# VideoVerses/VideoTuna-dev

Hardware: AMD Instinct MI355X
Metric: finetune samples/sec, CogVideoX-2B T2V LoRA 49x480x720 bf16 (higher is better)
Workload: dtype bf16; 1 GPU; CogVideoX-2B T2V LoRA finetune 49x480x720 (configs[1]): latents [4,13,16,60,90], text [4,226,4096], r=4 LoRA on to_q/k/v/out, 4 samples per optimizer step as in the YAML (batch_size 2 x accumulate_grad_batches 2), run as 1 micro-batch(es) of 4; mode=lora, model=CogVideoX-2B, micro_batch=4, accumulate_grad_batches=1, global_batch=4, seq_len=17776, layers=30, parallelism=dp1, recompute=none (107 GB of block activations kept in HBM), weights=seeded random init (no checkpoints offline), text=pre-encoded prompt embeddings (synthetic), latents=pre-encoded latents (synthetic)

## Files before the change

### include/vt355.h

```cpp
#ifndef VT355_H
#define VT355_H
#ifdef __cplusplus
extern "C" {
#endif

#define VT_OK 0
#define VT_ERR_BAD_SHAPE (-1)
#define VT_ERR_BAD_ALIGN (-2)
#define VT_ERR_LAUNCH (-3)
#define VT_ERR_UNSUPPORTED (-4)

int vt_version(void);
const char* vt_arch(void);
const char* vt_error_string(int code);

#define VT_EPI_BIAS 0
#define VT_EPI_BIAS_GELU 1
#define VT_EPI_GATED_RES 2
#define VT_EPI_DGELU 3

int vt_gemm_bf16(const void* A, int lda, const void* W, int ldw, void* C, int ldc,
                 int M, int N, int K, const void* bias, int epilogue, int out_fp32,
                 const void* R, int ldr, int r_mod,
                 const float* gate_txt, const float* gate_vid, int gate_bstride, int S, int St,
                 void* C2, int ldc2, const void* U, int ldu, void* stream);
int vt_gemm_set_tile(int mode);
int vt_gemm_bf16_kernel(int M, int N, int K);
int vt_conv_set_tile(int mode);

int vt_gemm_nt_bf16(const void* A, int lda, const void* B, int ldb, float* C, int ldc, int M, int P, int Q,
                    float alpha, int accumulate, void* stream);
int vt_gemm_nt_bf16_unpad(const void* A, int lda, const void* B, int ldb, float* C, int ldc, int M, int P, int Q,
                          float alpha, int accumulate, int row_group, int row_keep, int col_group, int col_keep, void* stream);

int vt_group_colsum(const void* X, int ldx, const void* Y, int ldy, const float* mean, const float* rstd,
                    float* out1, float* out2, long long M, int D, int S, int St, int grouped,
                    long long o_bstride, long long o_segstride, void* stream);

int vt_qk_ln_param_grads(const float* dq_hat, int lddq, const void* dk_hat, int lddk, const void* qkv, int ld,
                         const float* mean, const float* rstd, float* out_2x2x64, long long M, int H,
                         const float* rope_cos, const float* rope_sin, int S, int St, void* stream);
int vt_ln_param_combine(const float* G1, const float* G2, int G, int D, const void* gamma, const void* beta,
                        const float* scale_txt, const float* scale_vid, int bstride, float* dgamma, float* dbeta,
                        float* dshift_txt, float* dshift_vid, float* dscale_txt, float* dscale_vid, int dbstride,
                        int grouped, void* stream);
int vt_small_linear_bwd(const float* dy, int ldy, const void* x, int ldx, const void* W, float* dW, float* db,
                        float* dx, int lddx, int Bn, int N, int K, void* stream);
int vt_silu_bwd(const float* dy, const void* x, float* dx, long long n, void* stream);

int vt_attn_fwd_hd64(const void* q, const void* k, const void* v, void* o, float* lse2,
                     int B, int H, int S,
                     long long q_rs, long long k_rs, long long v_rs, long long o_rs,
                     long long q_bs, long long k_bs, long long v_bs, long long o_bs,
                     float softmax_scale, int q_prescaled, void* stream);

int vt_attn_fwd_bias_hd64(const void* q, const void* k, const void* v, const float* bias_t, void* o, float* lse2,
                          int B, int H, int S,
                          long long q_rs, long long k_rs, long long v_rs, long long o_rs,
                          long long q_bs, long long k_bs, long long v_bs, long long o_bs,
                          float softmax_scale, void* stream);
int vt_gemm_splitk_f32(const void* A, int lda, const void* W, int ldw, float* C, int ldc, int M, int N, int K, int splits, void* stream);
int vt_residual_cast_bf16(const float* acc, long long lda, const void* R, long long ldr, void* out, long long ldo, long long M, int N,
                          void* stream);
long long vt_groupnorm_ws_bytes(int N, int C);
int vt_groupnorm_silu_cl(const void* x, long long ldx, const void* gamma, const void* beta, void* y, long long ldy,
                         int N, long long P, int C, int G, float eps, int silu, float* ws, long long ws_bytes, void* stream);
int vt_causal_conv3d_cl(const void* x, long long ldx, const void* wk, const void* bias, const void* res, long long ldr,
                        void* y, long long ldy, int N, int T, int H, int W, int Cin, int Cout, void* stream);
int vt_downsample_conv2d_cl(const void* x, long long ldx, const void* wk, const void* bias, void* y, long long ldy,
                            int N, int T, int H, int W, int Cin, int Cout, void* stream);
int vt_causal_conv3d_in8_cl(const void* x, const void* wk, const void* bias, void* y, long long ldy,
                            int N, int T, int H, int W, int Cout, void* stream);
int vt_temporal_pool_cl(const void* x, long long ldx, void* y, long long ldy, int N, int T, long long HW, int C, int keep_first,
                        void* stream);
int vt_rmsnorm_bf16(const void* x, long long ldx, const void* w, void* y, long long ldy, long long M, int D, float eps,
                    void* stream);
int vt_gated_gelu_bf16(const void* u, long long ldu, void* y, long long ldy, long long M, int F, void* stream);

int vt_attn_bwd_hd64(const void* q, const void* k, const void* v, const void* o, const void* dout,
                     const float* lse2, float* delta_ws, float* dq_f32, void* dk, void* dv,
                     int B, int H, int S,
                     long long q_rs, long long k_rs, long long v_rs, long long o_rs, long long do_rs,
                     long long dq_rs, long long dk_rs, long long dv_rs,
                     long long q_bs, long long k_bs, long long v_bs, long long o_bs, long long do_bs,
                     long long dq_bs, long long dk_bs, long long dv_bs,
                     float softmax_scale, int q_prescaled, void* chain_ws, long long chain_ws_bytes, void* stream);
long long vt_attn_bwd_chain_ws_bytes(int B, int H, int S);
int vt_attn_bwd_set_chain(int chain_len, int slots);

int vt_ln_modulate_fwd(const void* x, int ldx, void* y, int ldy, const void* gamma, const void* beta,
                       const float* shift_txt, const float* scale_txt, const float* shift_vid,
                       const float* scale_vid, int mod_bstride, float* mean, float* rstd,
                       int M, int D, int S, int St, float eps, void* stream);
int vt_ln_modulate_bwd(const void* dy, int lddy, const void* x, int ldx, const float* mean, const float* rstd,
                       const void* gamma, const float* scale_txt, const float* scale_vid, int mod_bstride,
                       const void* dres, int lddres, void* dx, int lddx,
                       int M, int D, int S, int St, void* stream);

int vt_qk_layernorm_fwd(const void* qkv, int ld, void* out, int ldo, const void* gq, const void* bq,
                        const void* gk, const void* bk, float* mean, float* rstd,
                        long long M, int H, float eps, float q_scale,
                        const float* rope_cos, const float* rope_sin, int S, int St, void* stream);
int vt_qk_layernorm_bwd(const float* dq_hat, int lddq, const void* dk_hat, int lddk, const void* qkv, int ld,
                        const float* mean, const float* rstd, const void* gq, const void* gk,
                        void* dqkv, int ldd, long long M, int H,
                        const float* rope_cos, const float* rope_sin, int S, int St, void* stream);

int vt_gate_mul(const void* x, int ldx, void* y, int ldy, const float* g_txt, const float* g_vid, int bstride,
                long long M, int D, int S, int St, void* stream);
int vt_silu_bf16(const void* x, void* y, long long n, void* stream);
// ... 212 lines not shown
```

### videotuna-dev_amd/_lib.py

```python
import ctypes as C
import os

_HERE = os.path.dirname(os.path.abspath(__file__))
_LIB = None


class VtError(RuntimeError):
    pass


def lib_path() -> str:
    return os.environ.get("VT355_LIB") or os.path.join(_HERE, "libvt355.so")


_vp, _i, _ll, _f, _fp = C.c_void_p, C.c_int, C.c_longlong, C.c_float, C.c_void_p
PROTOTYPES = {
    "vt_version": [],
    "vt_arch": [],
    "vt_error_string": [_i],
    "vt_gemm_bf16": [_vp, _i, _vp, _i, _vp, _i, _i, _i, _i, _vp, _i, _i, _vp, _i, _i, _fp, _fp, _i, _i, _i,
                     _vp, _i, _vp, _i, _vp],
    "vt_gemm_set_tile": [_i],
    "vt_gemm_bf16_kernel": [_i, _i, _i],
    "vt_conv_set_tile": [_i],
    "vt_transpose_bf16": [_vp, _ll, _ll, _vp, _ll, _ll, _i, _i, _i, _vp],
    "vt_transpose_multi_bf16": [_vp, _i, _ll, _vp],
    "vt_gemm_nt_bf16": [_vp, _i, _vp, _i, _fp, _i, _i, _i, _i, _f, _i, _vp],
    "vt_gemm_nt_bf16_unpad": [_vp, _i, _vp, _i, _fp, _i, _i, _i, _i, _f, _i, _i, _i, _i, _i, _vp],
    "vt_group_colsum": [_vp, _i, _vp, _i, _fp, _fp, _fp, _fp, _ll, _i, _i, _i, _i, _ll, _ll, _vp],
    "vt_qk_ln_param_grads": [_fp, _i, _vp, _i, _vp, _i, _fp, _fp, _fp, _ll, _i, _fp, _fp, _i, _i, _vp],
    "vt_ln_param_combine": [_fp, _fp, _i, _i, _vp, _vp, _fp, _fp, _i, _fp, _fp, _fp, _fp, _fp, _fp, _i, _i, _vp],
    "vt_small_linear_bwd": [_fp, _i, _vp, _i, _vp, _fp, _fp, _fp, _i, _i, _i, _i, _vp],
    "vt_silu_bwd": [_fp, _vp, _fp, _ll, _vp],
    "vt_attn_fwd_hd64": [_vp, _vp, _vp, _vp, _fp, _i, _i, _i, _ll, _ll, _ll, _ll, _ll, _ll, _ll, _ll, _f, _i, _vp],
    "vt_attn_fwd_bias_hd64": [_vp, _vp, _vp, _fp, _vp, _fp, _i, _i, _i, _ll, _ll, _ll, _ll, _ll, _ll, _ll, _ll, _f, _vp],
    "vt_gemm_splitk_f32": [_vp, _i, _vp, _i, _fp, _i, _i, _i, _i, _i, _vp],
    "vt_residual_cast_bf16": [_fp, _ll, _vp, _ll, _vp, _ll, _ll, _i, _vp],
    "vt_groupnorm_ws_bytes": [_i, _i],
    "vt_groupnorm_silu_cl": [_vp, _ll, _vp, _vp, _vp, _ll, _i, _ll, _i, _i, _f, _i, _fp, _ll, _vp],
    "vt_causal_conv3d_cl": [_vp, _ll, _vp, _vp, _vp, _ll, _vp, _ll, _i, _i, _i, _i, _i, _i, _vp],
    "vt_causal_conv3d_in8_cl": [_vp, _vp, _vp, _vp, _ll, _i, _i, _i, _i, _i, _vp],
    "vt_downsample_conv2d_cl": [_vp, _ll, _vp, _vp, _vp, _ll, _i, _i, _i, _i, _i, _i, _vp],
    "vt_temporal_pool_cl": [_vp, _ll, _vp, _ll, _i, _i, _ll, _i, _i, _vp],
    "vt_rmsnorm_bf16": [_vp, _ll, _vp, _vp, _ll, _ll, _i, _f, _vp],
    "vt_gated_gelu_bf16": [_vp, _ll, _vp, _ll, _ll, _i, _vp],
    "vt_attn_bwd_hd64": [_vp, _vp, _vp, _vp, _vp, _fp, _fp, _fp, _vp, _vp, _i, _i, _i,
                         _ll, _ll, _ll, _ll, _ll, _ll, _ll, _ll, _ll, _ll, _ll, _ll, _ll, _ll, _ll, _ll, _f, _i, _vp, _ll, _vp],
    "vt_attn_bwd_chain_ws_bytes": [_i, _i, _i],
    "vt_attn_bwd_set_chain": [_i, _i],
    "vt_ln_modulate_fwd": [_vp, _i, _vp, _i, _vp, _vp, _fp, _fp, _fp, _fp, _i, _fp, _fp, _i, _i, _i, _i, _f, _vp],
    "vt_ln_modulate_bwd": [_vp, _i, _vp, _i, _fp, _fp, _vp, _fp, _fp, _i, _vp, _i, _vp, _i, _i, _i, _i, _i, _vp],
    "vt_qk_layernorm_fwd": [_vp, _i, _vp, _i, _vp, _vp, _vp, _vp, _fp, _fp, _ll, _i, _f, _f, _fp, _fp, _i, _i, _vp],
    "vt_qk_layernorm_bwd": [_fp, _i, _vp, _i, _vp, _i, _fp, _fp, _vp, _vp, _vp, _i, _ll, _i, _fp, _fp, _i, _i, _vp],
    "vt_gate_mul": [_vp, _i, _vp, _i, _fp, _fp, _i, _ll, _i, _i, _i, _vp],
    "vt_silu_bf16": [_vp, _vp, _ll, _vp],
    "vt_cast_f32_bf16": [_fp, _vp, _ll, _vp],
    "vt_timestep_embedding": [_vp, _vp, _i, _i, _i, _f, _vp],
    "vt_patchify": [_vp, _vp, _i, _i, _i, _i, _i, _i, _i, _vp],
    "vt_unpatchify": [_vp, _vp, _i, _i, _i, _i, _i, _i, _i, _vp],
    "vt_add_noise": [_fp, _fp, _fp, _fp, _vp, _ll, _i, _vp],
    "vt_diffusion_loss": [_vp, _vp, _fp, _fp, _fp, _fp, _fp, _fp, _vp, _ll, _i, _f, _vp],
    "vt_diffusion_loss_bwd": [_vp, _vp, _fp, _fp, _fp, _fp, _fp, _vp, _ll, _i, _vp],
    "vt_adamw": [_fp, _fp, _fp, _fp, _vp, _ll, _f, _f, _f, _f, _f, _i, _f, _vp, _vp],
    "vt_grad_sqnorm_partials": [],
    "vt_grad_sqnorm": [_fp, _ll, _fp, _i, _vp],
    "vt_clip_finalize": [_fp, _i, _f, _f, _fp, _vp],
    "vt_adamw_clip": [_fp, _fp, _fp, _fp, _vp, _ll, _f, _f, _f, _f, _f, _i, _f, _vp, _fp, _f, _vp],
    "vt_lora_down": [_vp, _i, _vp, _i, _i, _vp, _i, _ll, _i, _i, _vp],
    "vt_skinny_tn": [_vp, _i, _vp, _i, _i, _fp, _ll, _ll, _f, _ll, _i, _fp, _vp],
    "vt_skinny_tn_workspace_bytes": [_i],
    "vt_lora_up_add": [_vp, _i, _vp, _i, _vp, _i, _i, _ll, _i, _vp],
    "vt_lora_pack_b": [_fp, _vp, _i, _i, _i, _i, _f, _vp],
    "vt_lora_pack_bt": [_fp, _vp, _i, _i, _i, _i, _f, _vp],
    "vt_lora_down_wide": [_vp, _i, _vp, _i, _i, _i, _i, _i, _vp, _i, _ll, _i, _vp],
    "vt_lora_tn_wide": [_vp, _i, _vp, _i, _i, _fp, _ll, _ll, _f, _ll, _i, _vp],
    "vt_lora_up_add_wide": [_vp, _i, _vp, _i, _vp, _i, _i, _i, _i, _ll, _i, _vp],
    "vt_lora_pack_b_wide": [_fp, _vp, _i, _i, _i, _i, _i, _i, _f, _vp],
    "vt_lora_pack_bt_wide": [_fp, _vp, _i, _i, _i, _i, _i, _i, _f, _vp],
    "vt_lora_down_drop": [_vp, _i, _vp, _i, _i, _i, _vp, _i, _ll, _i, _i, _f, C.c_ulonglong, _i, _vp],
    "vt_skinny_tn_drop": [_vp, _i, _vp, _i, _i, _i, _fp, _ll, _ll, _f, _ll, _i, _fp, _f, C.c_ulonglong, _i, _vp],
    "vt_lora_up_add_drop": [_vp, _i, _vp, _i, _vp, _i, _i, _i, _ll, _i, _f, C.c_ulonglong, _i, _vp],
    "vt_lora_down_wide_drop_fits": [_i, _i],
    "vt_lora_down_wide_drop": [_vp, _i, _vp, _i, _i, _i, _i, _i, _vp, _i, _ll, _i, _f, C.c_ulonglong, _i, _vp],
    "vt_lora_tn_wide_drop": [_vp, _i, _vp, _i, _i, _fp, _ll, _ll, _f, _ll, _i, _f, C.c_ulonglong, _i, _vp],
    "vt_lora_up_add_wide_drop": [_vp, _i, _vp, _i, _vp, _i, _i, _i, _i, _ll, _i, _f, C.c_ulonglong, _i, _vp],
    "vt_lora_up_add_dgelu_drop": [_vp, _i, _vp, _i, _vp, _i, _i, _i, _vp, _i, _ll, _i, _f, C.c_ulonglong, _i, _vp],
    "vt_lora_up_add_wide_dgelu_drop": [_vp, _i, _vp, _i, _vp, _i, _i, _i, _i, _vp, _i, _ll, _i, _f, C.c_ulonglong, _i, _vp],
    "vt_lora_down_wide_drop_at": [_vp, _i, _vp, _i, _i, _i, _i, _i, _vp, _i, _ll, _i, _f, C.c_ulonglong, _i] + [_ll] * 5 + [_i, _i, _vp],
    "vt_lora_tn_wide_drop_at": [_vp, _i, _vp, _i, _i, _fp, _ll, _ll, _f, _ll, _i, _f, C.c_ulonglong, _i] + [_ll] * 5 + [_i, _i, _vp],
    "vt_lora_up_add_wide_drop_at": [_vp, _i, _vp, _i, _vp, _i, _i, _i, _i, _ll, _i, _f, C.c_ulonglong, _i] + [_ll] * 5 + [_i, _i, _vp],
    "vt_lora_up_add_wide_dgelu_drop_at": [_vp, _i, _vp, _i, _vp, _i, _i, _i, _i, _vp, _i, _ll, _i, _f, C.c_ulonglong, _i] + [_ll] * 5
                                         + [_i, _i, _vp],
    "vt_dora_norm": [_vp, _i, _vp, _i, _vp, _i, _i, _i, _i, _f, _fp, _fp, _vp],
    "vt_dora_scale": [_vp, _ll, _vp, _ll, _fp, _i, _i, _i, _vp],
    "vt_dora_transpose_scale": [_vp, _ll, _vp, _ll, _fp, _i, _i, _vp],
    "vt_dora_db_add": [_fp, _fp, _fp, _i, _i, _vp],
    "vt_dora_dm": [_fp, _fp, _vp, _fp, _fp, _i, _vp],
    "vt_conv_cl": [_vp, _ll, _vp, _vp, _fp, _i, _vp, _ll, _vp, _ll] + [_i] * 13 + [_vp],
    "vt_conv_dw_cl": [_vp, _ll, _vp, _ll, _fp] + [_i] * 13 + [_i, _vp],
    "vt_conv_dw_bias_cl": [_vp, _ll, _vp, _ll, _fp, _fp] + [_i] * 13 + [_i, _vp],
    "vt_conv_desc_extents": [_ll, _ll] + [_i] * 11 + [C.POINTER(C.c_longlong)] * 3,
    "vt_groupnorm_silu_bwd_cl": [_vp, _ll, _vp, _ll, _vp, _fp, _fp, _ll, _vp, _ll, _fp, _fp, _i, _ll, _i, _i, _i, _i, _vp],
    "vt_geglu_fwd": [_vp, _ll, _vp, _ll, _ll, _i, _vp],
    "vt_geglu_bwd": [_vp, _ll, _vp, _ll, _vp, _ll, _ll, _i, _vp],
    "vt_add_rows_bf16": [_vp, _ll, _vp, _ll, _vp, _ll, _ll, _i, _vp],
# ... 60 lines not shown
```

### videotuna-dev_amd/csrc/gemm_bf16.hip

```cpp
#include "gemm_epilogue.h"

#define BM 128
#define BN 128
#define BK 64
#define CS_LD 132

template <int EPI, bool OUT_F32>
__global__ __launch_bounds__(256, 2) void gemm_tn_kernel(GemmParams p) {
    __shared__ __attribute__((aligned(16))) char smem[65536];
    const int tid = threadIdx.x, lane = tid & 63, wave = tid >> 6;
    const int wm = wave & 1, wn = wave >> 1;
    const int nbm = (p.M + BM - 1) / BM, nbn = (p.N + BN - 1) / BN;
    const int id = xcd_remap(blockIdx.x, nbm * nbn);
    const int GM = 8;
    const int in_group = GM * nbn;
    const int group = id / in_group;
    const int first_m = group * GM;
    const int gsz = min(nbm - first_m, GM);
    const int tile_m = first_m + (id % in_group) % gsz;
    const int tile_n = (id % in_group) / gsz;
    const int row0 = tile_m * BM, col0 = tile_n * BN;

    const long long a_rem = (long long)(p.M - row0) * p.lda * 2;
    const long long w_rem = (long long)(p.N - col0) * p.ldw * 2;
// ... 36 lines not shown
        if (kt + 1 < nk) dma(kt + 1, buf ^ 1);
        const char* As = smem + buf * 32768;
        const char* Ws = As + 16384;
#pragma unroll
        for (int ks = 0; ks < 2; ++ks) {
            const int coff = (((ks * 4 + fq) ^ fx) << 4);
            bf16x8 af[4], wf[4];
#pragma unroll
            for (int t = 0; t < 4; ++t) {
                af[t] = *(const bf16x8*)(As + (wm * 64 + t * 16 + frow) * 128 + coff);
                wf[t] = *(const bf16x8*)(Ws + (wn * 64 + t * 16 + frow) * 128 + coff);
            }
#pragma unroll
            for (int tn = 0; tn < 4; ++tn)
#pragma unroll
                for (int tm = 0; tm < 4; ++tm)
                    acc[tn][tm] = __builtin_amdgcn_mfma_f32_16x16x32_bf16(wf[tn], af[tm], acc[tn][tm], 0, 0, 0);
        }
        __syncthreads();
    }

    float* Cs = (float*)smem;
    const int er = tid >> 5;
    const int ec = (tid & 31) * 4;
    const int n = col0 + ec;
    float bias4[4] = {0.f, 0.f, 0.f, 0.f};
    if (p.bias != nullptr && n < p.N) {
#pragma unroll
        for (int j = 0; j < 4; ++j) bias4[j] = bf2f(p.bias[n + j]);
    }
#pragma unroll
    for (int half = 0; half < 2; ++half) {
        if (wm == half) {
#pragma unroll
            for (int tn = 0; tn < 4; ++tn)
#pragma unroll
                for (int tm = 0; tm < 4; ++tm) {
                    int ml = tm * 16 + frow;
                    int nl = wn * 64 + tn * 16 + fq * 4;
                    *(f32x4*)(Cs + ml * CS_LD + nl) = acc[tn][tm];
                }
        }
        __syncthreads();
#pragma unroll
        for (int pass = 0; pass < 8; ++pass) {
            const int ml = pass * 8 + er;
            const int m = row0 + half * 64 + ml;
            if (m < p.M && n < p.N) {
                f32x4 v = *(const f32x4*)(Cs + ml * CS_LD + ec);
                gemm_epilogue_store<EPI, OUT_F32>(p, m, n, v, bias4);
            }
        }
        __syncthreads();
    }
}

template <int EPI, bool F32>
static int launch(const GemmParams& p, hipStream_t st) {
    const int nbm = (p.M + BM - 1) / BM, nbn = (p.N + BN - 1) / BN;
    hipLaunchKernelGGL((gemm_tn_kernel<EPI, F32>), dim3(nbm * nbn), dim3(256), 0, st, p);
    return hipGetLastError() == hipSuccess ? VT_OK : VT_ERR_LAUNCH;
}

static bool al16(const void* p) { return (((uintptr_t)p) & 15) == 0; }

int vt_gemm_big_dispatch(const GemmParams& p, int epilogue, int out_fp32, hipStream_t st);
int vt_gemm_pc_dispatch(const GemmParams& p, int epilogue, int out_fp32, hipStream_t st);
static int g_gemm_tile = 0;
extern "C" int vt_gemm_set_tile(int mode) {
    if (mode < 0 || mode > 3) return VT_ERR_BAD_SHAPE;
    g_gemm_tile = mode;
    return VT_OK;
}
static int pick_tile(int M, int N, int K) {
    const int mode = g_gemm_tile;
    if (mode) return mode;
    const long long t256 = (long long)((M + 255) / 256) * ((N + 255) / 256);
    const long long tpc = (long long)((M + 255) / 256) * ((N + 127) / 128);
    if (N >= 6144 && t256 >= 512) return 2;
    if (K >= 512 && M >= 1024) {
        const long long passes = (t256 + 255) / 256;
        const bool full = t256 <= 256 ? t256 >= 160 : 10 * t256 >= 9 * passes * 256;
        if (full && (N >= 2560 || ((N % 640) == 0 && N <= 1280) || ((N % 256) >= 192 && K >= 4096))) return 2;
    }
    if (tpc >= 512 && K >= 512) return 3;
    if (M > 64 && M <= 1024 && (long long)N * K >= (1LL << 24)) return 3;
    return 1;
}

int vt_gemm_pc_bm(int M);
extern "C" int vt_gemm_bf16_kernel(int M, int N, int K) {
    if (M <= 0 || N <= 0 || K <= 0) return VT_ERR_BAD_SHAPE;
    const int tile = pick_tile(M, N, K);
    return tile == 3 && vt_gemm_pc_bm(M) == 128 ? 4 : tile;
}

extern "C" int vt_gemm_bf16(const void* A, int lda, const void* W, int ldw, void* C, int ldc,
                            int M, int N, int K, const void* bias, int epilogue, int out_fp32,
                            const void* R, int ldr, int r_mod,
                            const float* gate_txt, const float* gate_vid, int gate_bstride, int S, int St,
                            void* C2, int ldc2, const void* U, int ldu, void* stream) {
    if (M <= 0 || N <= 0 || K <= 0 || (K % BK) != 0 || (N % 4) != 0) return VT_ERR_BAD_SHAPE;
    if ((lda % 8) || (ldw % 8) || (ldc % 4) || lda < K || ldw < K || ldc < N) return VT_ERR_BAD_SHAPE;
    if (!al16(A) || !al16(W) || !al16(C)) return VT_ERR_BAD_ALIGN;
    GemmParams p;
    p.A = (const bf16_t*)A; p.W = (const bf16_t*)W; p.C = C; p.bias = (const bf16_t*)bias;
    p.R = (const bf16_t*)R; p.gate_txt = gate_txt; p.gate_vid = gate_vid;
    p.C2 = (bf16_t*)C2; p.U = (const bf16_t*)U;
    p.M = M; p.N = N; p.K = K; p.lda = lda; p.ldw = ldw; p.ldc = ldc; p.ldr = ldr; p.ldc2 = ldc2; p.ldu = ldu;
    p.S = S > 0 ? S : 1; p.St = St; p.gate_bstride = gate_bstride; p.r_mod = r_mod; p.splits = 1;
    hipStream_t st = (hipStream_t)stream;
    const int tile = pick_tile(M, N, K);
    const bool big = tile == 2;
    if (tile == 3) {
        if (epilogue == EPI_BIAS_GELU && (out_fp32 || C2 == nullptr || (ldc2 % 4) || !al16(C2))) return VT_ERR_BAD_SHAPE;
        if (epilogue == EPI_GATED_RES && (out_fp32 || R == nullptr || (ldr % 4) || !al16(R))) return VT_ERR_BAD_SHAPE;
        if (epilogue == EPI_DGELU && (out_fp32 || U == nullptr || (ldu % 4) || !al16(U))) return VT_ERR_BAD_SHAPE;
        return vt_gemm_pc_dispatch(p, epilogue, out_fp32, st);
    }
    switch (epilogue) {
        case EPI_BIAS:
            if (big) return vt_gemm_big_dispatch(p, epilogue, out_fp32, st);
            return out_fp32 ? launch<EPI_BIAS, true>(p, st) : launch<EPI_BIAS, false>(p, st);
        case EPI_BIAS_GELU:
            if (out_fp32 || C2 == nullptr || (ldc2 % 4) || !al16(C2)) return VT_ERR_BAD_SHAPE;
            if (big) return vt_gemm_big_dispatch(p, epilogue, 0, st);
            return launch<EPI_BIAS_GELU, false>(p, st);
        case EPI_GATED_RES:
            if (out_fp32 || R == nullptr || (ldr % 4) || !al16(R)) return VT_ERR_BAD_SHAPE;
            if (C2 != nullptr && ((ldc2 % 4) || !al16(C2))) return VT_ERR_BAD_SHAPE;
            if (gate_vid != nullptr && (gate_txt == nullptr || (gate_bstride % 4) || !al16(gate_vid) || !al16(gate_txt)))
                return VT_ERR_BAD_SHAPE;
            if (big) return vt_gemm_big_dispatch(p, epilogue, 0, st);
            return launch<EPI_GATED_RES, false>(p, st);
        case EPI_DGELU:
            if (out_fp32 || U == nullptr || (ldu % 4) || !al16(U)) return VT_ERR_BAD_SHAPE;
            if (big) return vt_gemm_big_dispatch(p, epilogue, 0, st);
            return launch<EPI_DGELU, false>(p, st);
        default:
            return VT_ERR_UNSUPPORTED;
    }
}
```

### videotuna-dev_amd/csrc/gemm_big_bf16.hip

```cpp
#include "gemm_epilogue.h"

#define GB_BM 256
#define GB_BN 256
#define GB_BK 64
#define GB_STAGE 65536
#define GB_CS_LD 260

typedef int gb_i32x4 __attribute__((ext_vector_type(4)));

__device__ __forceinline__ gb_i32x4 gb_words(const void* base, unsigned bytes) {
    const unsigned long long a = (unsigned long long)base;
    return (gb_i32x4){(int)(unsigned)a, (int)((a >> 32) & 0xffffu), (int)bytes, 0x00020000};
}

template <int EPI, bool OUT_F32>
__global__ __launch_bounds__(512, 1) void gemm_tn_big_kernel(GemmParams p) {
    __shared__ __attribute__((aligned(16))) char smem[2 * GB_STAGE];
    const int tid = threadIdx.x, lane = tid & 63;
    const int wave = __builtin_amdgcn_readfirstlane(tid >> 6);
    const int wm = wave & 1, wn = wave >> 1;
    const int nbm = (p.M + GB_BM - 1) / GB_BM, nbn = (p.N + GB_BN - 1) / GB_BN;
    const int ntiles = nbm * nbn;
    const int spx = gridDim.x >> 3;
    const int slot = (int)(blockIdx.x & 7) * spx + (int)(blockIdx.x >> 3);
    const unsigned smem_lds = (unsigned)(uintptr_t)(__attribute__((address_space(3))) char*)smem;

    const int drl = lane >> 3, dcp = lane & 7;
    const int row0p = 8 * wave + drl;
    const int sw = (row0p >> 1) & 7;
    const int a_voff0 = row0p * p.lda * 2 + ((dcp ^ sw) << 4);
    const int w_voff0 = row0p * p.ldw * 2 + ((dcp ^ sw) << 4);
    const int a_pstep = 64 * p.lda * 2, w_pstep = 64 * p.ldw * 2;
    auto dma = [&](const GemmTile& t, int kt, int buf) {
        const int soff = kt * GB_BK * 2;
        __amdgpu_buffer_rsrc_t ra = make_rsrc(t.a, t.a_bytes), rw = make_rsrc(t.w, t.w_bytes);
#pragma unroll
        for (int j = 0; j < 4; ++j) {
            char* dst = smem + buf * GB_STAGE + (wave + 8 * j) * 1024;
            __builtin_amdgcn_raw_ptr_buffer_load_lds(ra, (__attribute__((address_space(3))) void*)dst, 16, a_voff0, soff + j * a_pstep, 0, 0);
            __builtin_amdgcn_raw_ptr_buffer_load_lds(rw, (__attribute__((address_space(3))) void*)(dst + 32768), 16, w_voff0, soff + j * w_pstep, 0, 0);
        }
    };
    auto dma_hidden = [&](const GemmTile& t, int buf) {
        const gb_i32x4 ra = gb_words(t.a, t.a_bytes), rw = gb_words(t.w, t.w_bytes);
#pragma unroll
        for (int j = 0; j < 4; ++j) {
            const unsigned dst = smem_lds + buf * GB_STAGE + (wave + 8 * j) * 1024;
            asm volatile("s_mov_b32 m0, %0\n\ts_nop 0\n\tbuffer_load_dwordx4 %1, %2, %3 offen lds" :: "s"(dst), "v"(a_voff0), "s"(ra), "s"(j * a_pstep) : "memory");
            asm volatile("s_mov_b32 m0, %0\n\ts_nop 0\n\tbuffer_load_dwordx4 %1, %2, %3 offen lds" :: "s"(dst + 32768), "v"(w_voff0), "s"(rw), "s"(j * w_pstep) : "memory");
        }
    };

    const int nk = p.K / GB_BK;
    const int fr16 = lane & 15, fq = lane >> 4, fx16 = (fr16 >> 1) & 7;
    const int er = tid >> 6;
    const int ec = (tid & 63) * 4;

    if (slot >= ntiles) return;
    GemmTile cur = gemm_tile<GB_BM, GB_BN>(p, slot, nbm, nbn);
    int buf = 0;
    dma(cur, 0, 0);
    for (int tile = slot; tile < ntiles; tile += gridDim.x) {
        const bool has_next = tile + (int)gridDim.x < ntiles;
        GemmTile nxt = cur;
        if (has_next) nxt = gemm_tile<GB_BM, GB_BN>(p, tile + gridDim.x, nbm, nbn);

        f32x4 acc16[4][8];
#pragma unroll
        for (int i = 0; i < 4; ++i)
#pragma unroll
            for (int j = 0; j < 8; ++j) acc16[i][j] = (f32x4){0.f, 0.f, 0.f, 0.f};

        __syncthreads();
        for (int kt = 0; kt < nk; ++kt) {
            const bool last = kt + 1 == nk;
            auto issue = [&]() {
                if (!last) dma(cur, kt + 1, buf ^ 1);
                else if (has_next) dma_hidden(nxt, buf ^ 1);
            };
            const bool late = wave >= 4;
            if (!late) issue();
            const char* As = smem + buf * GB_STAGE + (wm * 128 + fr16) * 128;
            const char* Ws = smem + buf * GB_STAGE + 32768 + (wn * 64 + fr16) * 128;
#pragma unroll
            for (int ks = 0; ks < 2; ++ks) {
                if (ks == 1 && late) issue();
                const int coff = (((ks * 4 + fq) ^ fx16) << 4);
                bf16x8 af[8], wf[4];
#pragma unroll
                for (int t = 0; t < 8; ++t) af[t] = *(const bf16x8*)(As + t * 2048 + coff);
#pragma unroll
                for (int t = 0; t < 4; ++t) wf[t] = *(const bf16x8*)(Ws + t * 2048 + coff);
#pragma unroll
                for (int tm = 0; tm < 8; ++tm)
#pragma unroll
                    for (int tn = 0; tn < 4; ++tn)
                        acc16[tn][tm] = __builtin_amdgcn_mfma_f32_16x16x32_bf16(wf[tn], af[tm], acc16[tn][tm], 0, 0, 0);
            }
            if (!last) __syncthreads();
            else gemm_lds_barrier();
            buf ^= 1;
        }

        float* Cs = (float*)(smem + (buf ^ 1) * GB_STAGE);
        const int n = cur.col0 + ec;
        float bias4[4] = {0.f, 0.f, 0.f, 0.f};
        if (p.bias != nullptr && n < p.N) {
#pragma unroll
            for (int j = 0; j < 4; ++j) bias4[j] = bf2f(p.bias[n + j]);
        }
        constexpr bool HAS_AUX = EPI == EPI_GATED_RES || EPI == EPI_DGELU;
        u32x2 aux[4], auxn[4];
        auto aux_fetch = [&](int slab, u32x2* dst) {
#pragma unroll
            for (int pass = 0; pass < 4; ++pass) {
                const int m = cur.row0 + slab * 32 + pass * 8 + er;
                dst[pass] = (u32x2){0u, 0u};
                if (HAS_AUX && wave < 8 && m < p.M && n < p.N) dst[pass] = gemm_epilogue_aux_load<EPI>(p, m, n);
            }
        };
        aux_fetch(0, aux);
        GateCtx gctx;
        if (EPI == EPI_GATED_RES) gctx = gate_ctx_load(p, cur.row0, GB_BM, n);
#pragma unroll
        for (int slab = 0; slab < 8; ++slab) {
            if (wave < 8 && wm == (slab >> 2)) {
#pragma unroll
                for (int t2 = 0; t2 < 2; ++t2)
#pragma unroll
                    for (int tn = 0; tn < 4; ++tn)
                        *(f32x4*)(Cs + (t2 * 16 + fr16) * GB_CS_LD + wn * 64 + tn * 16 + 4 * fq) = acc16[tn][(slab & 3) * 2 + t2];
            }
            gemm_lds_barrier();
            if (slab < 7) aux_fetch(slab + 1, auxn);
#pragma unroll
            for (int pass = 0; pass < 4; ++pass) {
                const int ml = pass * 8 + er;
                const int m = cur.row0 + slab * 32 + ml;
                if (wave < 8 && m < p.M && n < p.N) {
                    const f32x4 v = *(const f32x4*)(Cs + ml * GB_CS_LD + ec);
                    gemm_epilogue_store_aux<EPI, OUT_F32>(p, m, n, v, bias4, aux[pass], EPI == EPI_GATED_RES ? &gctx : nullptr);
                }
            }
            gemm_lds_barrier();
#pragma unroll
            for (int pass = 0; pass < 4; ++pass) aux[pass] = auxn[pass];
        }
        cur = nxt;
    }
}

template <int EPI, bool F32>
static int launch_big(const GemmParams& p, hipStream_t st) {
    const int nbm = (p.M + GB_BM - 1) / GB_BM, nbn = (p.N + GB_BN - 1) / GB_BN;
    static int slots = 0;
    if (slots == 0) {
        int dev = 0, cus = 0;
        if (hipGetDevice(&dev) != hipSuccess || hipDeviceGetAttribute(&cus, hipDeviceAttributeMultiprocessorCount, dev) != hipSuccess) cus = 0;
        slots = cus >= 8 ? cus / 8 * 8 : 8;
    }
    const int ntiles = nbm * nbn;
    const int grid = ntiles < slots ? (ntiles + 7) / 8 * 8 : slots;
    hipLaunchKernelGGL((gemm_tn_big_kernel<EPI, F32>), dim3(grid), dim3(512), 0, st, p);
    return hipGetLastError() == hipSuccess ? VT_OK : VT_ERR_LAUNCH;
}

int vt_gemm_big_dispatch(const GemmParams& p, int epilogue, int out_fp32, hipStream_t st) {
    switch (epilogue) {
        case EPI_BIAS:
            return out_fp32 ? launch_big<EPI_BIAS, true>(p, st) : launch_big<EPI_BIAS, false>(p, st);
        case EPI_BIAS_GELU: return launch_big<EPI_BIAS_GELU, false>(p, st);
        case EPI_GATED_RES: return launch_big<EPI_GATED_RES, false>(p, st);
        case EPI_DGELU: return launch_big<EPI_DGELU, false>(p, st);
        default: return VT_ERR_UNSUPPORTED;
    }
}
```

### videotuna-dev_amd/ops.py

```python
from __future__ import annotations

import math
import os
from typing import Optional

import torch

from ._lib import check, load_library

BF16 = torch.bfloat16
EPI_BIAS, EPI_BIAS_GELU, EPI_GATED_RES, EPI_DGELU = 0, 1, 2, 3


def _stream() -> int:
    return torch.cuda.current_stream().cuda_stream


_PROFILE = {"on": False, "events": {}, "work": {}}
_PROFILED = ("attn_fwd", "attn_bwd", "conv", "conv_dw")


def profile_reset(on: bool):
    _PROFILE["on"] = on
    if on:
# ... 304 lines not shown
    check(load_library().vt_downsample_conv2d_cl(x.data_ptr(), x.stride(3), wk.data_ptr(), _p(bias), y.data_ptr(), y.stride(3),
                                                 N, T, H, W, Cin, Cout, _stream()), "vt_downsample_conv2d_cl")
    return y


def temporal_pool_frames(T: int, keep_first: bool) -> int:
    return 1 + (T - 1) // 2 if keep_first else T // 2


def temporal_pool(x, y, keep_first: bool = True):
    _req(x, BF16, "x", 5); _req(y, BF16, "y", 5)
    N, T, H, W, C = x.shape
    To = temporal_pool_frames(T, keep_first)
    if tuple(y.shape) != (N, To, H, W, C) or To < 1:
        raise ValueError(f"y must be {(N, To, H, W, C)}, got {tuple(y.shape)}")
    _cl_check(x, "x"); _cl_check(y, "y")
    check(load_library().vt_temporal_pool_cl(x.data_ptr(), x.stride(3), y.data_ptr(), y.stride(3), N, T, H * W, C, int(keep_first),
                                             _stream()), "vt_temporal_pool_cl")
    return y


def rmsnorm(x, w, y, eps: float = 1e-6):
    _req(x, BF16, "x", 2); _req(y, BF16, "y", 2); _req(w, BF16, "w", 1)
    check(load_library().vt_rmsnorm_bf16(x.data_ptr(), x.stride(0), w.data_ptr(), y.data_ptr(), y.stride(0), x.shape[0], x.shape[1],
                                         eps, _stream()), "vt_rmsnorm_bf16")


def gated_gelu(u, y):
    _req(u, BF16, "u", 2); _req(y, BF16, "y", 2)
    check(load_library().vt_gated_gelu_bf16(u.data_ptr(), u.stride(0), y.data_ptr(), y.stride(0), u.shape[0], y.shape[1], _stream()),
          "vt_gated_gelu_bf16")


def attn_bwd_chain_workspace(B: int, H: int, S: int, device) -> Optional[torch.Tensor]:
    if _SIDE_STREAMS["n"] > 0 or _CHAIN_STATE["disabled"]:
        return None
    n = int(load_library().vt_attn_bwd_chain_ws_bytes(B, H, S))
    if n <= 0:
        return None
    key = str(device)
    ws = _CHAIN_WS.get(key)
    if ws is None or ws.numel() < n:
        old = ws
        ws = _CHAIN_WS[key] = torch.empty(n, dtype=torch.uint8, device=device)
        ws[:256].zero_()
        if old is not None:
            ws[64:256].copy_(old[64:256])
    return ws


_CHAIN_WS = {}
_SIDE_STREAMS = {"n": 0}
_CHAIN_STATE = {"disabled": False, "redone": 0, "verify": __import__("os").environ.get("VT355_CHAIN_VERIFY", "launch")}


def attn_bwd_chain_redone() -> int:
    return _CHAIN_STATE["redone"]


def declare_side_stream(active: bool):
    _SIDE_STREAMS["n"] = max(0, _SIDE_STREAMS["n"] + (1 if active else -1))


def chain_guard(device) -> Optional[torch.Tensor]:
    ws = _CHAIN_WS.get(str(device))
    return None if ws is None else ws[64:68].view(torch.int32)


def attn_bwd_chain_errors() -> int:
    return sum(int(ws[64:68].view(torch.int32).item()) for ws in _CHAIN_WS.values())


def attn_bwd_chain_errors_clear():
    for ws in _CHAIN_WS.values():
        ws[64:256].zero_()


def conv_set_tile(mode: int = 0):
    check(load_library().vt_conv_set_tile(mode), "vt_conv_set_tile")


def gemm_set_tile(mode: int = 0):
    check(load_library().vt_gemm_set_tile(mode), "vt_gemm_set_tile")


def gemm_kernel(M: int, N: int, K: int) -> int:
    k = load_library().vt_gemm_bf16_kernel(M, N, K)
    if k < 0:
        check(k, "vt_gemm_bf16_kernel")
    return k


def attn_bwd_set_chain(chain_len: int = 0, slots: int = 0):
    check(load_library().vt_attn_bwd_set_chain(chain_len, slots), "vt_attn_bwd_set_chain")


def attn_bwd_chain_error(chain_ws: torch.Tensor) -> int:
    return int(chain_ws[32:36].view(torch.int32).item())


def attn_bwd(q, k, v, o, do, lse2, delta_ws, dq_f32, dk, dv, B: int, H: int, S: int, scale: Optional[float] = None,
             q_prescaled: bool = False, chain_ws: Optional[torch.Tensor] = None, _entry=None):
    scale = 1.0 / math.sqrt(64) if scale is None else scale
    for n, t in (("q", q), ("k", k), ("v", v), ("o", o), ("do", do), ("dk", dk), ("dv", dv)):
        _req(t, BF16, n, 3)
    _req(dq_f32, torch.float32, "dq_f32", 3)
    lib = load_library()

    def launch(ws, fn=None):
        check((fn or lib.vt_attn_bwd_hd64)(q.data_ptr(), k.data_ptr(), v.data_ptr(), o.data_ptr(), do.data_ptr(),
                               lse2.data_ptr(), delta_ws.data_ptr(), dq_f32.data_ptr(), dk.data_ptr(), dv.data_ptr(),
                               B, H, S,
                               q.stride(1), k.stride(1), v.stride(1), o.stride(1), do.stride(1),
                               dq_f32.stride(1), dk.stride(1), dv.stride(1),
                               q.stride(0), k.stride(0), v.stride(0), o.stride(0), do.stride(0),
                               dq_f32.stride(0), dk.stride(0), dv.stride(0), scale, int(q_prescaled),
                               None if ws is None else ws.data_ptr(), 0 if ws is None else ws.numel(),
                               _stream()),
          "vt_attn_bwd_hd64")
    with _timed("attn_bwd"):
        launch(chain_ws, _entry)
    if chain_ws is not None and _CHAIN_STATE["verify"] == "launch" and attn_bwd_chain_error(chain_ws) != 0:
        import warnings
        _CHAIN_STATE["disabled"] = True
        _CHAIN_STATE["redone"] += 1
        warnings.warn("vt_attn_bwd_hd64: a dQ hand-off wait timed out (the persistent workgroups were not all resident: another stream or a "
                      "profiler shared the CUs); the launch was redone with plain atomics and the hand-off chains are switched off for the rest "
                      "of this process (VT_BWD_CHAIN=1 avoids them from the start; ops.declare_side_stream(True) announces a concurrent stream)")
        dq_f32.zero_()
        launch(None)
        chain_ws[32:36].zero_()
        chain_ws[64:68].zero_()


def ln_modulate_fwd(x, y, gamma, beta, mod, mean, rstd, D: int, S: int, St: int, eps: float):
    _req(x, BF16, "x", 2); _req(y, BF16, "y", 2)
    m = (None, None, None, None, 0) if mod is None else mod
    lib = load_library()
    with _timed_hbm("ln_modulate_fwd", x.shape[0], 4.0 * x.shape[0] * D):
        check(lib.vt_ln_modulate_fwd(x.data_ptr(), x.stride(0), y.data_ptr(), y.stride(0), _p(gamma), _p(beta),
                                     _p(m[0]), _p(m[1]), _p(m[2]), _p(m[3]), m[4], _p(mean), _p(rstd),
                                     x.shape[0], D, S, St, eps, _stream()), "vt_ln_modulate_fwd")


def ln_modulate_bwd(dy, x, mean, rstd, gamma, scales, dres, dx, D: int, S: int, St: int):
    _req(dy, BF16, "dy", 2); _req(x, BF16, "x", 2); _req(dx, BF16, "dx", 2)
    sc = (None, None, 0) if scales is None else scales
    lib = load_library()
    with _timed_hbm("ln_modulate_bwd", x.shape[0], (6.0 if dres is None else 8.0) * x.shape[0] * D):
        check(lib.vt_ln_modulate_bwd(dy.data_ptr(), dy.stride(0), x.data_ptr(), x.stride(0), mean.data_ptr(), rstd.data_ptr(),
                                     _p(gamma), _p(sc[0]), _p(sc[1]), sc[2], _p(dres), 0 if dres is None else dres.stride(0),
                                     dx.data_ptr(), dx.stride(0), x.shape[0], D, S, St, _stream()), "vt_ln_modulate_bwd")


def qk_layernorm_fwd(qkv, out, gq, bq, gk, bk, mean, rstd, H: int, eps: float, q_scale: float = 1.0, rope=None):
    _req(qkv, BF16, "qkv", 2); _req(out, BF16, "out", 2)
    lib = load_library()
    rc, rsn, S, St = _rope_args(rope, qkv.shape[0])
    with _timed_hbm("qk_layernorm_fwd", qkv.shape[0], 8.0 * qkv.shape[0] * H * 64):
        check(lib.vt_qk_layernorm_fwd(qkv.data_ptr(), qkv.stride(0), out.data_ptr(), out.stride(0), gq.data_ptr(), bq.data_ptr(),
                                      gk.data_ptr(), bk.data_ptr(), mean.data_ptr(), rstd.data_ptr(), qkv.shape[0], H, eps,
                                      q_scale, rc, rsn, S, St, _stream()), "vt_qk_layernorm_fwd")


def qk_layernorm_bwd(dq_hat_f32, dk_hat, qkv, mean, rstd, gq, gk, dqkv, H: int, rope=None):
    _req(dq_hat_f32, torch.float32, "dq_hat", 2); _req(dk_hat, BF16, "dk_hat", 2)
# ... 985 lines not shown
```

Measured before the change: 2.851 samples/s.

## Add phased quadrant K-loop to big GEMM and widen big-tile selection

Adds a PHASED variant of the 256x256 big GEMM kernel. It splits each K-tile into four MFMA quadrants, interleaves per-quadrant LDS fragment reads and half-tile buffer_load-to-LDS prefetches between them, staggers the two wave halves with an extra barrier, and raises wave priority during MFMA bursts. The aim is to overlap global loads and LDS reads with matrix math better than the single per-K-tile barrier loop did. The tile picker also routes more K<4096 shapes with mostly-full waves to the big kernel. This adds intricate waitcnt and barrier accounting that risks hangs or races on edge shapes.

```diff
diff --git a/include/vt355.h b/include/vt355.h
--- a/include/vt355.h
+++ b/include/vt355.h
@@ -26,6 +26,7 @@
                  void* C2, int ldc2, const void* U, int ldu, void* stream);
 int vt_gemm_set_tile(int mode);
 int vt_gemm_bf16_kernel(int M, int N, int K);
+int vt_gemm_set_big_loop(int mode);
 int vt_conv_set_tile(int mode);
 
 int vt_gemm_nt_bf16(const void* A, int lda, const void* B, int ldb, float* C, int ldc, int M, int P, int Q,
diff --git a/videotuna-dev_amd/_lib.py b/videotuna-dev_amd/_lib.py
--- a/videotuna-dev_amd/_lib.py
+++ b/videotuna-dev_amd/_lib.py
@@ -21,6 +21,7 @@
     "vt_gemm_bf16": [_vp, _i, _vp, _i, _vp, _i, _i, _i, _i, _vp, _i, _i, _vp, _i, _i, _fp, _fp, _i, _i, _i,
                      _vp, _i, _vp, _i, _vp],
     "vt_gemm_set_tile": [_i],
+    "vt_gemm_set_big_loop": [_i],
     "vt_gemm_bf16_kernel": [_i, _i, _i],
     "vt_conv_set_tile": [_i],
     "vt_transpose_bf16": [_vp, _ll, _ll, _vp, _ll, _ll, _i, _i, _i, _vp],
diff --git a/videotuna-dev_amd/csrc/gemm_bf16.hip b/videotuna-dev_amd/csrc/gemm_bf16.hip
--- a/videotuna-dev_amd/csrc/gemm_bf16.hip
+++ b/videotuna-dev_amd/csrc/gemm_bf16.hip
@@ -142,6 +142,9 @@
         const long long passes = (t256 + 255) / 256;
         const bool full = t256 <= 256 ? t256 >= 160 : 10 * t256 >= 9 * passes * 256;
         if (full && (N >= 2560 || ((N % 640) == 0 && N <= 1280) || ((N % 256) >= 192 && K >= 4096))) return 2;
+        const long long nbn = (N + 255) / 256;
+        const bool most = t256 > 256 && 100 * t256 >= 85 * passes * 256;
+        if ((full || most) && K < 4096 && 16LL * N >= 15 * 256 * nbn) return 2;
     }
     if (tpc >= 512 && K >= 512) return 3;
     if (M > 64 && M <= 1024 && (long long)N * K >= (1LL << 24)) return 3;
diff --git a/videotuna-dev_amd/csrc/gemm_big_bf16.hip b/videotuna-dev_amd/csrc/gemm_big_bf16.hip
--- a/videotuna-dev_amd/csrc/gemm_big_bf16.hip
+++ b/videotuna-dev_amd/csrc/gemm_big_bf16.hip
@@ -13,7 +13,7 @@
     return (gb_i32x4){(int)(unsigned)a, (int)((a >> 32) & 0xffffu), (int)bytes, 0x00020000};
 }
 
-template <int EPI, bool OUT_F32>
+template <int EPI, bool OUT_F32, bool PHASED>
 __global__ __launch_bounds__(512, 1) void gemm_tn_big_kernel(GemmParams p) {
     __shared__ __attribute__((aligned(16))) char smem[2 * GB_STAGE];
     const int tid = threadIdx.x, lane = tid & 63;
@@ -51,6 +51,15 @@
         }
     };
 
+    auto half = [&](const gb_i32x4 ra, const gb_i32x4 rw, int kt, int b, int h) {
+        const unsigned dst = smem_lds + b * GB_STAGE + wave * 1024 + (h >= 2 ? 32768 : 0);
+        const int j0 = h == 0 ? 0 : h == 1 ? 1 : h == 2 ? 0 : 2, j1 = h == 0 ? 2 : h == 1 ? 3 : h == 2 ? 1 : 3;
+        const int soff = kt * GB_BK * 2, pstep = h >= 2 ? w_pstep : a_pstep, voff = h >= 2 ? w_voff0 : a_voff0;
+        const gb_i32x4 rs = h >= 2 ? rw : ra;
+        asm volatile("s_mov_b32 m0, %0\n\ts_nop 0\n\tbuffer_load_dwordx4 %1, %2, %3 offen lds" :: "s"(dst + j0 * 8192), "v"(voff), "s"(rs), "s"(soff + j0 * pstep) : "memory");
+        asm volatile("s_mov_b32 m0, %0\n\ts_nop 0\n\tbuffer_load_dwordx4 %1, %2, %3 offen lds" :: "s"(dst + j1 * 8192), "v"(voff), "s"(rs), "s"(soff + j1 * pstep) : "memory");
+    };
+
     const int nk = p.K / GB_BK;
     const int fr16 = lane & 15, fq = lane >> 4, fx16 = (fr16 >> 1) & 7;
     const int er = tid >> 6;
@@ -59,7 +68,12 @@
     if (slot >= ntiles) return;
     GemmTile cur = gemm_tile<GB_BM, GB_BN>(p, slot, nbm, nbn);
     int buf = 0;
+    if constexpr (PHASED) {
+#pragma unroll
+        for (int h = 0; h < 4; ++h) half(gb_words(cur.a, cur.a_bytes), gb_words(cur.w, cur.w_bytes), 0, 0, h);
+    } else {
     dma(cur, 0, 0);
+    }
     for (int tile = slot; tile < ntiles; tile += gridDim.x) {
         const bool has_next = tile + (int)gridDim.x < ntiles;
         GemmTile nxt = cur;
@@ -71,6 +85,7 @@
 #pragma unroll
             for (int j = 0; j < 8; ++j) acc16[i][j] = (f32x4){0.f, 0.f, 0.f, 0.f};
 
+        if constexpr (!PHASED) {
         __syncthreads();
         for (int kt = 0; kt < nk; ++kt) {
             const bool last = kt + 1 == nk;
@@ -101,6 +116,107 @@
             else gemm_lds_barrier();
             buf ^= 1;
         }
+        } else {
+        const bool late = wave >= 4;
+        const gb_i32x4 ra_c = gb_words(cur.a, cur.a_bytes), rw_c = gb_words(cur.w, cur.w_bytes);
+        const gb_i32x4 ra_n = gb_words(nxt.a, nxt.a_bytes), rw_n = gb_words(nxt.w, nxt.w_bytes);
+        {
+            const bool own = nk > 1;
+            if (own || has_next) {
+                half(own ? ra_c : ra_n, own ? rw_c : rw_n, own ? 1 : 0, buf ^ 1, 0);
+                half(own ? ra_c : ra_n, own ? rw_c : rw_n, own ? 1 : 0, buf ^ 1, 2);
+                half(own ? ra_c : ra_n, own ? rw_c : rw_n, own ? 1 : 0, buf ^ 1, 3);
+                asm volatile("s_waitcnt vmcnt(6)" ::: "memory");
+            } else {
+                asm volatile("s_waitcnt vmcnt(0)" ::: "memory");
+            }
+            asm volatile("s_barrier" ::: "memory");
+            if (late) asm volatile("s_barrier" ::: "memory");
+        }
+        bf16x8 fa[4][2], fw0[2][2], fw1[2][2];
+        auto read_a = [&](const char* As, int qa) {
+#pragma unroll
+            for (int t = 0; t < 4; ++t)
+#pragma unroll
+                for (int ks = 0; ks < 2; ++ks) fa[t][ks] = *(const bf16x8*)(As + (qa * 4 + t) * 2048 + (((ks * 4 + fq) ^ fx16) << 4));
+        };
+        auto read_w = [&](const char* Ws, int qw, bf16x8 (&fw)[2][2]) {
+#pragma unroll
+            for (int t = 0; t < 2; ++t)
+#pragma unroll
+                for (int ks = 0; ks < 2; ++ks) fw[t][ks] = *(const bf16x8*)(Ws + (qw * 2 + t) * 2048 + (((ks * 4 + fq) ^ fx16) << 4));
+        };
+        auto mfma_head = [&]() {
+            asm volatile("s_waitcnt lgkmcnt(0)" ::: "memory");
+            asm volatile("s_barrier" ::: "memory");
+            __builtin_amdgcn_sched_barrier(0);
+            __builtin_amdgcn_s_setprio(1);
+        };
+        auto mfma_tail = [&]() {
+            __builtin_amdgcn_s_setprio(0);
+            __builtin_amdgcn_sched_barrier(0);
+            asm volatile("s_barrier" ::: "memory");
+        };
+#define GB_QUADRANT(QA, QW, FW)                                                                                                   \
+    _Pragma("unroll") for (int ks = 0; ks < 2; ++ks)                                                                               \
+    _Pragma("unroll") for (int t = 0; t < 4; ++t)                                                                                  \
+    _Pragma("unroll") for (int u = 0; u < 2; ++u)                                                                                  \
+        acc16[(QW) * 2 + u][(QA) * 4 + t] = __builtin_amdgcn_mfma_f32_16x16x32_bf16(FW[u][ks], fa[t][ks], acc16[(QW) * 2 + u][(QA) * 4 + t], 0, 0, 0);
+        auto ktile = [&](int kt, int b, auto steady) {
+            constexpr bool STEADY = decltype(steady)::value;
+            const bool own1 = STEADY || kt + 1 < nk, own2 = STEADY || kt + 2 < nk;
+            const bool i1 = own1 || has_next;
+            const bool i2 = own2 || (kt + 2 == nk && has_next);
+            const gb_i32x4 ra1 = own1 ? ra_c : ra_n, ra2 = own2 ? ra_c : ra_n, rw2 = own2 ? rw_c : rw_n;
+            const int k1 = own1 ? kt + 1 : 0, k2 = own2 ? kt + 2 : 0;
+            const char* As = smem + b * GB_STAGE + (wm * 128 + fr16) * 128;
+            const char* Ws = smem + b * GB_STAGE + 32768 + (wn * 64 + fr16) * 128;
+            read_w(Ws, 0, fw0);
+            __builtin_amdgcn_sched_barrier(0);
+            read_a(As, 0);
+            __builtin_amdgcn_sched_barrier(0);
+            if (i1) half(ra1, ra1, k1, b ^ 1, 1);
+            mfma_head();
+            GB_QUADRANT(0, 0, fw0)
+            mfma_tail();
+            read_w(Ws, 1, fw1);
+            __builtin_amdgcn_sched_barrier(0);
+            if (i2) half(ra2, rw2, k2, b, 0);
+            mfma_head();
+            GB_QUADRANT(0, 1, fw1)
+            mfma_tail();
+            read_a(As, 1);
+            __builtin_amdgcn_sched_barrier(0);
+            if (i2) half(ra2, rw2, k2, b, 2);
+            mfma_head();
+            GB_QUADRANT(1, 1, fw1)
+            mfma_tail();
+            if (i2) half(ra2, rw2, k2, b, 3);
+            if (STEADY || kt + 1 < nk) {
+                if (i2) asm volatile("s_waitcnt vmcnt(6)" ::: "memory");
+                else asm volatile("s_waitcnt vmcnt(0)" ::: "memory");
+            }
+            mfma_head();
+            GB_QUADRANT(1, 0, fw0)
+            mfma_tail();
+        };
+        int kt = 0;
+        for (; kt + 4 <= nk; kt += 2) {
+            ktile(kt, buf, std::true_type());
+            ktile(kt + 1, buf ^ 1, std::true_type());
+        }
+        if (kt + 3 <= nk) {
+            ktile(kt, buf, std::true_type());
+            ++kt;
+            buf ^= 1;
+        }
+        for (; kt < nk; ++kt) {
+            ktile(kt, buf, std::false_type());
+            buf ^= 1;
+        }
+        if (!late) asm volatile("s_barrier" ::: "memory");
+#undef GB_QUADRANT
+        }
 
         float* Cs = (float*)(smem + (buf ^ 1) * GB_STAGE);
         const int n = cur.col0 + ec;
@@ -148,6 +264,18 @@
         }
         cur = nxt;
     }
+}
+
+static int g_big_loop = 0;
+extern "C" int vt_gemm_set_big_loop(int mode) {
+    if (mode < 0 || mode > 2) return VT_ERR_BAD_SHAPE;
+    g_big_loop = mode;
+    return VT_OK;
+}
+static bool big_loop_phased(const GemmParams& p) {
+    if (g_big_loop) return g_big_loop == 2;
+    const int nk = p.K / GB_BK;
+    return nk >= 8 || (nk >= 2 && p.N >= 2560);
 }
 
 template <int EPI, bool F32>
@@ -161,7 +289,8 @@
     }
     const int ntiles = nbm * nbn;
     const int grid = ntiles < slots ? (ntiles + 7) / 8 * 8 : slots;
-    hipLaunchKernelGGL((gemm_tn_big_kernel<EPI, F32>), dim3(grid), dim3(512), 0, st, p);
+    if (big_loop_phased(p)) hipLaunchKernelGGL((gemm_tn_big_kernel<EPI, F32, true>), dim3(grid), dim3(512), 0, st, p);
+    else hipLaunchKernelGGL((gemm_tn_big_kernel<EPI, F32, false>), dim3(grid), dim3(512), 0, st, p);
     return hipGetLastError() == hipSuccess ? VT_OK : VT_ERR_LAUNCH;
 }
 
diff --git a/videotuna-dev_amd/ops.py b/videotuna-dev_amd/ops.py
--- a/videotuna-dev_amd/ops.py
+++ b/videotuna-dev_amd/ops.py
@@ -410,6 +410,10 @@
 
 def gemm_set_tile(mode: int = 0):
     check(load_library().vt_gemm_set_tile(mode), "vt_gemm_set_tile")
+
+
+def gemm_set_big_loop(mode: int = 0):
+    check(load_library().vt_gemm_set_big_loop(mode), "vt_gemm_set_big_loop")
 
 
 def gemm_kernel(M: int, N: int, K: int) -> int:
```

Result: faster. 2.923 samples/s, median of 6 (+2.5%).
